# carry4985/ORB_SLAM2_MAP

Hardware: AMD Instinct MI355X
Metric: frames/sec ORB extract+match (640x480, 1000 feat) (higher is better)
Workload: dtype u8; 1 GPU; C2: synthetic 640x480 RGB-D stream, 1000 features, 8 levels, extract + BF-Hamming match of consecutive frames; resident_frame_pool=1024, sequences=1, parallelism=1 sequence per GPU, schedule_name=best, extraction_parts=1

## Files before the change

orb_slam2_map_amd/csrc/extractor.hip:

```cpp
#include "common.h"

#include <atomic>
#include <chrono>
#include <thread>
#include <tuple>
#include <type_traits>
#include <utility>
#include "trig_base.h"
#include "pyramid_view.h"
#include "extractor_plan.h"

#include <algorithm>
#include <cfloat>
#include <cmath>
#include <cstdlib>
#include <cstring>
#include <vector>

namespace orbgpu {

__host__ __device__ __forceinline__ uint32_t pack_key(int x, int y, int resp)
{
    return ((uint32_t)y << 20) | ((uint32_t)x << 8) | (uint32_t)resp;
}
// ... 1395 lines not shown
        best_done = last_pass;
        labelled = labelled || !last_pass;
        {
            int *t = S.ccnt;
            S.ccnt = S.ccnt_next;
            S.ccnt_next = t;
        }
        {
            short4 *tb = bndA; bndA = bndB; bndB = tb;
            int *tc = cntA; cntA = cntB; cntB = tc;
            uint16_t *tr = creA; creA = creB; creB = tr;
            uint32_t *tm = midA; midA = midB; midB = tm;
        }
        __syncthreads();
    }

    QT_MARK(3)
    const int n = n_cur;
    unsigned long long *best = reinterpret_cast<unsigned long long *>(S.ccnt);
    if (!best_done) {
        for (int p = tid; p < n; p += nt)
            best[p] = 0ull;
        __syncthreads();
        for (int i0 = tid; i0 < nkeys; i0 += QT_ILP * nt) {
            uint32_t key[QT_ILP];
            int nd[QT_ILP];
#pragma unroll
            for (int u = 0; u < QT_ILP; u++) {
                const int i = min(i0 + u * nt, nkeys - 1);
                key[u] = key_at(i);
                nd[u] = node_of(i, key[u]);
            }
#pragma unroll
            for (int u = 0; u < QT_ILP; u++)
                if (i0 + u * nt < nkeys)
                    atomicMax(&best[nd[u]], best_of(key[u]));
        }
    }
    __syncthreads();
    uint32_t *osel = sel + (size_t)f * sel_cap_total + g.sel_off;
    const bool ok = done_cur != 2 && n <= g.sel_cap;
    for (int p = tid; p < n && ok; p += nt) {
        const unsigned long long b = best[p];
        const uint32_t yx = (uint32_t)((0xFFFFFFFFFFull - (b & 0xFFFFFFFFFFull)) & 0xFFFFFFull);
        osel[p] = (yx << 8) | (uint32_t)((b >> 40) - 1ull);
    }
    QT_MARK(4)
    if (tid == 0)
        nsel[(size_t)f * nlevels + level] = ok ? n : -1;
}

struct KpAux {
    int x, y, level;
    float angle;
    float ca, sb;
    int plane_off, pitch;
};

__device__ __forceinline__ float fast_atan2_deg(float y, float x)
{
    const float s = (float)(180 / 3.14159265358979323846);
    const float p1 = 0.9997878412794807f * s, p3 = -0.3258083974640975f * s;
    const float p5 = 0.1555786518463281f * s, p7 = -0.04432655554792128f * s;
    const float ax = fabsf(x), ay = fabsf(y);
    float a, c, c2;
    if (ax >= ay) {
        c = ay / (ax + (float)DBL_EPSILON);
        c2 = c * c;
        a = (((p7 * c2 + p5) * c2 + p3) * c2 + p1) * c;
    } else {
        c = ax / (ay + (float)DBL_EPSILON);
        c2 = c * c;
        a = 90.f - (((p7 * c2 + p5) * c2 + p3) * c2 + p1) * c;
    }
    if (x < 0)
        a = 180.f - a;
    if (y < 0)
        a = 360.f - a;
    return a;
}

constexpr int OR_ITERS = 4;
constexpr int OR_BATCH_MIN = 32;

__global__ __launch_bounds__(256) void k_orient(const uint8_t *__restrict__ pyr, size_t frame_pyr,
                                                const LevelGeom *__restrict__ geom, int nlevels,
                                                const uint32_t *__restrict__ sel, int sel_cap_total,
                                                const int *__restrict__ nsel, const uint32_t *__restrict__ orw,
                                                orbgpu_keypoint *__restrict__ kps, KpAux *__restrict__ aux,
                                                int cap, int *__restrict__ n_out, int iters, Src0 s0)
{
    __shared__ uint32_t W10[4 * 16 * 9], M01[4 * 16 * 9];
    __shared__ __align__(16) uint8_t stage[8][31 * 48];
    for (int i = threadIdx.x; i < 4 * 16 * 9; i += 256) {
        W10[i] = orw[i];
        M01[i] = orw[4 * 16 * 9 + i];
    }
    __syncthreads();

    const int hl = threadIdx.x & 31;
    int bx, f;
    xcd_frame_block(bx, f);
    f = serpentine(f);
    const int *ns = nsel + (size_t)f * nlevels;
    for (int it = 0; it < iters; it++) {
    const int slot = (bx * iters + it) * 8 + (threadIdx.x >> 5);
    int level = -1, j = 0, out_off = 0, total = 0, cnt_l = 0;
    bool bad = false;
    struct {
        int plane_off, pitch, sel_off, patch;
        float scale;
    } g = {0, 0, 0, 0, 1.f};
    for (int l = 0; l < nlevels; l++) {
        const int c = ns[l];
        if (c < 0)
            bad = true;
        const int so = geom[l].sel_off;
        if (slot >= so && slot < so + geom[l].sel_cap) {
            level = l;
            j = slot - so;
            out_off = total;
            cnt_l = c;
            g.plane_off = geom[l].plane_off;
            g.pitch = geom[l].pitch;
            g.sel_off = so;
            g.patch = geom[l].patch;
            g.scale = geom[l].scale;
        }
        total += max(c, 0);
    }
    if (slot == 0 && hl == 0)
        n_out[f] = bad ? -1 - total : (total > cap ? -1 - total : total);
    if (level < 0 || bad || total > cap || j >= cnt_l)
        continue;
    const uint32_t key = sel[(size_t)f * sel_cap_total + g.sel_off + j];
    const int x = key_x(key) + BORDER0, y = key_y(key) + BORDER0;
    const bool dir0 = s0.direct != 0 && level == 0;
    const int porg = dir0 ? 0 : EDGE, ppitch = dir0 ? (int)s0.pitch : g.pitch;
    const int xl = x + porg - HALF_PATCH;
    const int a = xl & 3;
    const int v = hl - HALF_PATCH;
    int m10 = 0, m01 = 0;
    {
        const uint8_t *base = (dir0 ? s0.p + (size_t)f * s0.frame_stride : pyr + (size_t)f * frame_pyr + g.plane_off) + (xl - a);
        struct __attribute__((packed, aligned(4))) Piece {
            uint32_t d[4];
        };
        const int lim = a == 2 ? 3 : (a == 3 ? 6 : -1);
        const uint8_t *rowbase = base + rowoff(y + porg - HALF_PATCH, ppitch);
        uint4 *pl = reinterpret_cast<uint4 *>(stage[threadIdx.x >> 5]);
        Piece pc[3];
#pragma unroll
        for (int k = 0; k < 2; k++) {
            const int q = hl + 32 * k, r = q >> 1, part = q & 1;
            if (q < 62)
                pc[k] = *reinterpret_cast<const Piece *>(rowbase + rowoff(r, ppitch) + part * 16);
        }
        const int r2 = HALF_PATCH - lim + hl;
        if (hl < 2 * lim + 1)
            pc[2] = *reinterpret_cast<const Piece *>(rowbase + rowoff(r2, ppitch) + 32);
#pragma unroll
        for (int k = 0; k < 2; k++) {
            const int q = hl + 32 * k;
            if (q < 62)
                pl[3 * (q >> 1) + (q & 1)] = make_uint4(pc[k].d[0], pc[k].d[1], pc[k].d[2], pc[k].d[3]);
        }
        if (hl < 2 * lim + 1)
            pl[3 * r2 + 2] = make_uint4(pc[2].d[0], pc[2].d[1], pc[2].d[2], pc[2].d[3]);
        __builtin_amdgcn_fence(__ATOMIC_RELEASE, "wavefront");
        __builtin_amdgcn_wave_barrier();
        __builtin_amdgcn_fence(__ATOMIC_ACQUIRE, "wavefront");
        if (hl < 31) {
            const int av = v < 0 ? -v : v;
            const uint32_t *row = reinterpret_cast<const uint32_t *>(stage[threadIdx.x >> 5]) + hl * 12;
            const uint32_t *w = &W10[(a * 16 + av) * 9], *m = &M01[(a * 16 + av) * 9];
            uint32_t sw = 0, sm = 0;
#pragma unroll
            for (int q = 0; q < 9; q++) {
                const uint32_t d = row[q];
                sw = __builtin_amdgcn_udot4(d, w[q], sw, false);
                sm = __builtin_amdgcn_udot4(d, m[q], sm, false);
            }
            m10 = (int)sw - 16 * (int)sm;
            m01 = v * (int)sm;
        }
        __builtin_amdgcn_fence(__ATOMIC_RELEASE, "wavefront");
        __builtin_amdgcn_wave_barrier();
    }
#pragma unroll
    for (int off = 16; off > 0; off >>= 1) {
        m10 += __shfl_xor(m10, off, 64);
        m01 += __shfl_xor(m01, off, 64);
    }
    if (hl == 0) {
        const float angle = fast_atan2_deg((float)m01, (float)m10);
        orbgpu_keypoint kp;
        kp.x = (float)x;
        kp.y = (float)y;
        if (level != 0) {
            kp.x *= g.scale;
            kp.y *= g.scale;
        }
        kp.size = (float)g.patch;
        kp.angle = angle;
        kp.response = (float)key_resp(key);
        kp.octave = level;
        kp.class_id = -1;
        kps[(size_t)f * cap + out_off + j] = kp;
        KpAux ax;
        ax.x = x + (dir0 ? BLUR0_OX - EDGE : 0);
        ax.y = y;
        ax.level = level;
        ax.plane_off = g.plane_off;
        ax.pitch = g.pitch;
        ax.angle = angle;
        aux[(size_t)f * cap + out_off + j] = ax;
    }
    }
}
__global__ __launch_bounds__(256) void k_trig(KpAux *__restrict__ aux, const int *__restrict__ n_out, int cap, TrigTable tt)
{
    const int f = blockIdx.y;
    const int i = blockIdx.x * 256 + threadIdx.x;
    if (i >= n_out[f])
        return;
    KpAux *a = aux + (size_t)f * cap + i;
    const float factorPI = (float)(3.14159265358979323846 / 180.f);
    const float angle = a->angle * factorPI;
    float c, s;
    orbgpu_trig_device(angle, tt, &c, &s);
    a->ca = c;
    a->sb = s;
}

__device__ __forceinline__ void blur_hsum(uint32_t d0, uint32_t d1, uint32_t d2, uint32_t h[4])
{
#define W4(a, b, c, d) ((uint32_t)(a) | ((uint32_t)(b) << 8) | ((uint32_t)(c) << 16) | ((uint32_t)(d) << 24))
    h[0] = __builtin_amdgcn_udot4(d1, W4(55, 49, 34, 18), __builtin_amdgcn_udot4(d0, W4(0, 18, 34, 49), 0u, false), false);
    h[1] = __builtin_amdgcn_udot4(d2, W4(18, 0, 0, 0), __builtin_amdgcn_udot4(d1, W4(49, 55, 49, 34), __builtin_amdgcn_udot4(d0, W4(0, 0, 18, 34), 0u, false), false), false);
    h[2] = __builtin_amdgcn_udot4(d2, W4(34, 18, 0, 0), __builtin_amdgcn_udot4(d1, W4(34, 49, 55, 49), __builtin_amdgcn_udot4(d0, W4(0, 0, 0, 18), 0u, false), false), false);
    h[3] = __builtin_amdgcn_udot4(d2, W4(49, 34, 18, 0), __builtin_amdgcn_udot4(d1, W4(18, 34, 49, 55), 0u, false), false);
#undef W4
}

__device__ __forceinline__ uint32_t blur_vsum(const uint32_t A[4], const uint32_t C[4], const uint32_t E[4],
                                              const uint32_t F[4])
{
    const us2 K01 = {18, 34}, K23 = {49, 55}, K45 = {49, 34}, K6 = {0, 18};
    uint32_t sv[4];
#pragma unroll
    for (int p = 0; p < 4; p++) {
        uint32_t acc = __builtin_amdgcn_udot2(__builtin_bit_cast(us2, A[p]), K01, 32768u, false);
        acc = __builtin_amdgcn_udot2(__builtin_bit_cast(us2, C[p]), K23, acc, false);
        acc = __builtin_amdgcn_udot2(__builtin_bit_cast(us2, E[p]), K45, acc, false);
        sv[p] = __builtin_amdgcn_udot2(__builtin_bit_cast(us2, F[p]), K6, acc, false);
    }
    const us2 cap = {255, 255};
    const us2 lo = __builtin_elementwise_min(__builtin_bit_cast(us2, __builtin_amdgcn_perm(sv[1], sv[0], 0x07060302u)), cap);
    const us2 hi = __builtin_elementwise_min(__builtin_bit_cast(us2, __builtin_amdgcn_perm(sv[3], sv[2], 0x07060302u)), cap);
    return __builtin_amdgcn_perm(__builtin_bit_cast(uint32_t, hi), __builtin_bit_cast(uint32_t, lo), 0x06040200u);
}

__global__ __launch_bounds__(256) void k_blur(const uint8_t *__restrict__ pyr, uint8_t *__restrict__ blur,
                                               size_t frame_pyr, const LevelGeom *__restrict__ geom, StripGeom bg, int strip0)
{
    int bx, f;
    xcd_frame_block(bx, f);
    f = serpentine(f);
    const int strip = strip0 + bx * 256 + threadIdx.x;
    if (strip >= bg.first[bg.nlevels])
        return;
    int level = 0;
#pragma unroll
    for (int l = 1; l < ORBGPU_MAX_LEVELS; l++)
        level += (l < bg.nlevels && strip >= bg.first[l]) ? 1 : 0;
    const LevelGeom g = geom[level];
    const int local = strip - bg.first[level];
    const int sy = local / bg.nsx[level], sx = local - sy * bg.nsx[level];
    const int col = (4 + 2 * sx) * 4;
    const int y0 = sy * BLUR_ROWS;
    const int rows = min(BLUR_ROWS, g.h - y0);
    const uint8_t *fsrc = pyr + (size_t)f * frame_pyr;
    uint8_t *fdst = blur + (size_t)f * frame_pyr;
    const uint32_t pitch = (uint32_t)g.pitch;
    const uint32_t src0 = (uint32_t)g.plane_off + (uint32_t)(y0 + EDGE - 3) * pitch + (uint32_t)(col - 4);
    uint32_t soff = src0 + 6u * pitch;
    uint32_t doff = (uint32_t)g.plane_off + (uint32_t)(y0 + EDGE) * pitch + (uint32_t)col;
    struct __attribute__((packed, aligned(4))) Q4 {
        uint32_t d[4];
    };
    uint32_t p0[8], p1[8], p2[8], p3[8], p4[8], p5[8], hn[8];
    Q4 nx;
#define B8_HSUM(R, Q)                                                                                        \
    {                                                                                                        \
        blur_hsum(Q.d[0], Q.d[1], Q.d[2], R);                                                                \
        blur_hsum(Q.d[1], Q.d[2], Q.d[3], R + 4);                                                            \
    }
#define B8_PAIR(P, PREV, H)                                                                                  \
    _Pragma("unroll") for (int p = 0; p < 8; p++) P[p] = __builtin_amdgcn_alignbit(H[p], PREV[p], 16);
#define B8_LOAD(P, PREV, row)                                                                                \
// ... 528 lines not shown
        if (!direct) {
            int rcb = materialize_level0(e, s0, batch, L);
            if (rcb != ORBGPU_OK)
                return rcb;
        }
        for (int l = 1; l < nl; l++) {
            const LevelGeom &gl = e->plan.geom[l];
            const ResizeLaunch rl = resize_launch(e->plan, l, batch, direct);
            if (rl.px == 8) {
                dim3 gr8((resize_n8(gl.w) * ((gl.h + rl.rows - 1) / rl.rows) + 255) / 256, batch);
                L.launch(rl.dir1 ? (rl.share ? k_resize_fast<true, true, 8, true> : k_resize_fast<true, true, 8, false>)
                                 : (rl.share ? k_resize_fast<true, false, 8, true> : k_resize_fast<true, false, 8, false>), gr8, dim3(256), 0, pyr,
                         e->plan.frame_pyr, dg, l, e->tab<ResizeStrip>(e->plan.t_r8item), e->tab<uint4>(e->plan.t_r8sel), e->tab<uint4>(e->plan.t_r8wt),
                         e->tab<YRow>(e->plan.t_yrow), rl.off, rl.rows, s0);
            } else if (rl.px == 4) {
                dim3 grf((resize_ndw(gl.w) * ((gl.h + rl.rows - 1) / rl.rows) + 255) / 256, batch);
                auto kern = rl.dir1 ? (rl.rows == PYR_ROWS ? k_resize_fast<true, true, 4> : k_resize_fast<false, true, 4>)
                                    : (rl.rows == PYR_ROWS ? k_resize_fast<true, false, 4> : k_resize_fast<false, false, 4>);
                L.launch(kern, grf, dim3(256), 0, pyr, e->plan.frame_pyr, dg, l, e->tab<ResizeStrip>(e->plan.t_rstrip),
                                   e->tab<uint4>(e->plan.t_rsel), e->tab<uint4>(e->plan.t_rwt), e->tab<YRow>(e->plan.t_yrow),
                                   rl.off, rl.rows, s0);
            } else {
                dim3 gr((gl.pitch / 4 + 255) / 256, gl.h + 2 * EDGE, batch);
                L.launch(k_resize_level, gr, dim3(256), 0, pyr, e->plan.frame_pyr, dg, l,
                                   e->tab<XTab>(e->plan.t_xtab), e->tab<YTab>(e->plan.t_ytab));
            }
        }
    }
    END(ST_PYRAMID, st);
    BEGIN(ST_BLUR, st);
    if (side_blur) {
        ORBGPU_HIP_TRY(hipEventRecord(e->ev_fork, st));
        ORBGPU_HIP_TRY(hipStreamWaitEvent(e->side, e->ev_fork, 0));
        if (prof && !early_blur0)
            ORBGPU_HIP_TRY(hipEventRecord(evs[ST_COUNT + 1], e->side));
        launch_blur(e, s0, batch, Ls, early_blur0 ? 2 : 0);
        if (prof)
            ORBGPU_HIP_TRY(hipEventRecord(evs[ST_COUNT + 2], e->side));
        ORBGPU_HIP_TRY(hipEventRecord(e->ev_join, e->side));
    } else
        launch_blur(e, s0, batch, L);
    END(ST_BLUR, st);
    BEGIN(ST_FAST, st);
    if (e->counters_dirty) {
        int rcm = L.memset32(e->d_cellcnt.p, e->d_cellcnt.bytes & ~(size_t)3);
        if (rcm == ORBGPU_OK)
            rcm = L.memset32(e->d_qtaux.p, e->d_qtaux.bytes & ~(size_t)3);
        if (rcm != ORBGPU_OK)
            return rcm;
    }
    e->counters_dirty = true;
    {
        const int t_ini = std::max(e->prm.ini_th_fast, 1), t_min = std::max(e->prm.min_th_fast, 1);
        const DetectGeom &dgeo = direct ? e->plan.det_geom_direct : e->plan.det_geom;
        const int nwaves = (dgeo.first[nl] + FD_OWN - 1) / FD_OWN;
        L.launch(e->fast_early_out ? k_fast_detect<true> : k_fast_detect<false>, dim3((nwaves + 3) / 4, batch), dim3(256), 0, pyr, e->plan.frame_pyr, dg,
                           dgeo, e->tab<ColumnInfo>(e->plan.t_ctab), e->tab<CellDesc>(e->plan.t_cells), e->plan.ncells,
                           e->d_slots.as<uint32_t>(), e->plan.frame_slots, e->d_cellcnt.as<int>(), std::min(t_ini, t_min),
                           t_ini, e->fast_queue_cap, s0);
    }
    END(ST_FAST, st);
    BEGIN(ST_QUADTREE, st);
    {
        const QuadtreeLaunch ql = quadtree_launch(e->plan, batch, e->force_batch_quadtree);
        const bool pre = ql.lds_keys && e->plan.qt_prefilter;
        if (pre)
            L.launch(k_qt_prefilter, dim3(std::min((e->plan.max_slots_level + QT_PRE_KEYS - 1) / QT_PRE_KEYS, QT_PRE_GRID), nl, batch), dim3(256), 0, dg, e->plan.ncells, e->d_slots.as<uint32_t>(), e->plan.frame_slots, e->d_cellcnt.as<int>(),
                               e->d_dkey.as<uint32_t>(), e->d_qtaux.as<int>(), std::max(e->prm.ini_th_fast, 1));
        L.launch(ql.lds_keys ? k_quadtree<true> : k_quadtree<false>, dim3(batch, nl), dim3(ql.threads), ql.lds_bytes, dg,
                           e->tab<CellDesc>(e->plan.t_cells), e->plan.ncells, e->d_slots.as<uint32_t>(), e->plan.frame_slots,
                           e->d_cellcnt.as<int>(), e->d_dkey.as<uint32_t>(), e->d_dnode.as<uint16_t>(),
                           e->d_sel.as<uint32_t>(), e->plan.sel_cap_total, e->d_nsel.as<int>(), e->d_ncand.as<int>(), nl,
                           e->plan.ncap, std::max(e->prm.ini_th_fast, 1), ql.kcap, qt_dbg(),
                           pre ? e->d_qtaux.as<int>() : (int *)nullptr);
    }
    if (!rec)
        ORBGPU_HIP_TRY(hipGetLastError());
    e->counters_dirty = false;
    END(ST_QUADTREE, st);
    BEGIN(ST_ORIENT, st);
    const int or_iters = batch >= OR_BATCH_MIN ? OR_ITERS : 1;
    L.launch(k_orient, dim3((e->plan.sel_cap_total + 8 * or_iters - 1) / (8 * or_iters), batch), dim3(256), 0, pyr, e->plan.frame_pyr, dg, nl,
                       e->d_sel.as<uint32_t>(), e->plan.sel_cap_total, e->d_nsel.as<int>(),
                       e->tab<uint32_t>(e->plan.t_orient), d_kps,
                       e->d_aux.as<KpAux>(), cap, d_n_out, or_iters, s0);
    L.launch(k_trig, dim3((std::min(cap, e->plan.max_kp) + 255) / 256, batch), dim3(256), 0,
                       e->d_aux.as<KpAux>(), d_n_out, cap, e->trig);
    END(ST_ORIENT, st);
    BEGIN(ST_DESCRIBE, st);
    if (side_blur)
        ORBGPU_HIP_TRY(hipStreamWaitEvent(st, e->ev_join, 0));
    L.launch(k_describe, dim3((std::min(cap, e->plan.max_kp) + 7) / 8, batch), dim3(256), 0, blur,
                       e->plan.frame_pyr, dg, e->d_aux.as<KpAux>(), d_n_out, cap, e->tab<int8_t>(e->plan.t_pattern), d_desc);
    END(ST_DESCRIBE, st);
#undef BEGIN
#undef END
    if (!rec)
        ORBGPU_HIP_TRY(hipGetLastError());
    else if (L.err != hipSuccess) {
        set_error("recording the extraction graph: %s", hipGetErrorString(L.err));
        return ORBGPU_EHIP;
    }
    if (prof)
        e->prof_calls++;
    (void)w;
    (void)h;
    return ORBGPU_OK;
}

}

namespace orbgpu {

int extractor_pyramid_view(const orbgpu_extractor *e, PyramidView *v)
{
    ORBGPU_REQUIRE(e && v, "null argument");
    memset(v, 0, sizeof(*v));
    v->device_id = e->prm.device_id;
    v->nlevels = e->nlevels;
    v->scale_factor = e->prm.scale_factor;
    v->last_batch = (int)e->plan.geom.size() == e->nlevels ? e->last.batch : 0;
    for (int l = 0; l < e->nlevels; l++) {
        v->scale[l] = e->consts.scale[l];
        v->inv_scale[l] = e->consts.inv_scale[l];
        if (v->last_batch > 0) {
            const LevelGeom &g = e->plan.geom[l];
            v->w[l] = g.w;
            v->h[l] = g.h;
            v->pitch[l] = g.pitch;
            v->plane_off[l] = g.plane_off;
        }
    }
    v->pyr = e->d_pyr.as<uint8_t>();
    v->frame_pyr = e->plan.frame_pyr;
    v->border = EDGE;
    v->direct = v->last_batch > 0 && e->last.src.direct ? 1 : 0;
    v->l0 = v->direct ? e->last.src.p : nullptr;
    v->l0_frame_stride = v->direct ? e->last.src.frame_stride : 0;
    v->l0_pitch = v->direct ? e->last.src.pitch : 0;
    v->scratch = &e->d_stereo;
    return ORBGPU_OK;
}

}

extern "C" {

static void free_handle(orbgpu_extractor *e)
{
    for (DevBuf *b : e->buffers())
        b->release();
    for (auto &x : e->ev)
        if (x)
            (void)hipEventDestroy(x);
    if (e->graph_exec)
        (void)hipGraphExecDestroy(e->graph_exec);
    if (e->graph)
        (void)hipGraphDestroy(e->graph);
    if (e->h_pin)
        (void)hipHostFree(e->h_pin);
    if (e->stream)
        (void)hipStreamDestroy(e->stream);
    if (e->side)
        (void)hipStreamDestroy(e->side);
    if (e->ev_fork)
        (void)hipEventDestroy(e->ev_fork);
    if (e->ev_fork0)
// ... 642 lines not shown
```

orb_slam2_map_amd/csrc/extractor_plan.h:

```cpp
#pragma once
#include <algorithm>
#include <cmath>
#include <cstdarg>
#include <cstdint>
#include <cstdio>
#include <cstdlib>
#include <cstring>
#include <string>
#include <utility>
#include <vector>

#include "orbgpu.h"
#include "resize_tables.h"

#ifdef __HIPCC__
#define ORBGPU_PLAN_HD __host__ __device__ __forceinline__
#else
#define ORBGPU_PLAN_HD inline
#endif

namespace orbgpu {

constexpr int EDGE = 19;
static_assert(EDGE == RS_EDGE, "resize_tables.h builds its tables for this border");
// ... 149 lines not shown
        desired *= factor;
    }
    c->quota[nl - 1] = std::max(nfeatures - sum, 0);

    int *um = c->umax.v;
    const int vmax = (int)floor(HALF_PATCH * sqrtf(2.f) / 2 + 1);
    const int vmin = (int)ceil(HALF_PATCH * sqrtf(2.f) / 2);
    const double hp2 = HALF_PATCH * HALF_PATCH;
    for (int v = 0; v <= vmax; ++v)
        um[v] = cv_round_host(sqrt(hp2 - v * v));
    for (int v = HALF_PATCH, v0 = 0; v >= vmin; --v) {
        while (um[v0] == um[v0 + 1])
            ++v0;
        um[v] = v0;
        ++v0;
    }
    static const int expect[16] = {15, 15, 15, 15, 14, 14, 14, 13, 13, 12, 11, 10, 9, 8, 6, 3};
    for (int v = 0; v <= HALF_PATCH; v++)
        ORBGPU_PLAN_REQUIRE(um[v] == expect[v], "umax[%d] = %d, k_orient is written for %d", v, um[v], expect[v]);
    return ORBGPU_OK;
}

struct LevelSize {
    int w, h;
    float width, height;
};
inline LevelSize level_size(const ExtractorConsts &c, int w, int h, int l)
{
    LevelSize s;
    s.w = cv_round_host((float)w * c.inv_scale[l]);
    s.h = cv_round_host((float)h * c.inv_scale[l]);
    s.width = (float)(s.w - 2 * BORDER0);
    s.height = (float)(s.h - 2 * BORDER0);
    return s;
}
inline int level_n_ini(const LevelSize &s) { return (int)roundf(s.width / s.height); }
inline int level_max_keypoints(int n_ini, int quota) { return std::max(4 * n_ini, quota + 3); }

inline RingGeom ring_geom(const std::vector<LevelGeom> &geom, int ring)
{
    RingGeom rg = {};
    rg.nlevels = (int)geom.size();
    for (int l = 1; l < rg.nlevels; l++)
        rg.first[l + 1] = rg.first[l] + 2 * ring * (geom[l].w + 2 * ring) + 2 * ring * geom[l].h;
    return rg;
}

static const int8_t k_pattern_host[1024] = {
#include "orbgpu_pattern.inc"
};

struct PlanHooks {
    int qt_keys = -1;
    bool qt_no_prefilter = false;
};

struct PlanTable {
    size_t off = 0, bytes = 0;
};
constexpr size_t PLAN_ALIGN = 256;

struct ExtractorPlan {
    int w = 0, h = 0;
    std::vector<LevelGeom> geom;
    int ncells = 0;
    StripGeom blur_geom = {};
    DetectGeom det_geom = {}, det_geom_direct = {};
    RingGeom ring_full = {};
    size_t frame_pyr = 0, frame_slots = 0;
    int sel_cap_total = 0, ncap = 0, max_kp = 0;
    size_t qt_lds = 0;
    int qt_kcap = 0;
    int max_slots_level = 0;
    bool qt_prefilter = false;
    bool border_fast = false;
    bool direct0_ok = false;
    int rs_off_direct = 0;
    int r8_off[ORBGPU_MAX_LEVELS] = {};
    int r8_off_direct = -1;
    bool r8_share[ORBGPU_MAX_LEVELS] = {}, r8_share_direct = false;
    bool interior_resize = false;
    std::vector<uint8_t> blob;
    PlanTable t_geom, t_cells, t_ctab, t_bcol, t_xtab, t_ytab, t_yrow, t_rstrip, t_rsel, t_rwt, t_r8item, t_r8sel, t_r8wt,
        t_pattern, t_orient;
    template <typename T> const T *table(const PlanTable &t) const { return reinterpret_cast<const T *>(blob.data() + t.off); }
    template <typename T> size_t count(const PlanTable &t) const { return t.bytes / sizeof(T); }
};

template <typename T> inline PlanTable plan_add_table(std::vector<uint8_t> &blob, const T *data, size_t n)
{
    PlanTable t;
    t.off = (blob.size() + PLAN_ALIGN - 1) / PLAN_ALIGN * PLAN_ALIGN;
    t.bytes = n * sizeof(T);
    blob.resize(t.off + t.bytes, 0);
    if (t.bytes)
        memcpy(blob.data() + t.off, data, t.bytes);
    return t;
}

inline bool plan_detect(const std::vector<LevelGeom> &geom, bool direct0, DetectGeom &dgm, std::vector<ColumnInfo> &ctab)
{
    const int nl = (int)geom.size();
    memset(&dgm, 0, sizeof(dgm));
    dgm.nlevels = nl;
    int acc = 0;
    for (int l = 0; l < nl; l++) {
        const LevelGeom &g = geom[l];
        const bool dir = direct0 && l == 0;
        const int xfirst = dir ? 16 : 9 * 4 - EDGE;
        const int nsx = dir ? (g.w - 20 - xfirst) / 4 + 1 : (g.w - 1) / 4 - 9 + 1;
        const int nbands = (g.h - 2 * EDGE + g.hcell - 1) / g.hcell;
        dgm.first[l] = acc;
        dgm.nsx[l] = nsx;
        dgm.ncols[l] = g.ncols_eff;
        dgm.ctab_off[l] = (int)ctab.size();
        dgm.xfirst[l] = xfirst;
        acc += nsx * nbands;
        if (dir)
            acc = (acc + FD_OWN - 1) / FD_OWN * FD_OWN;
        for (int sx = 0; sx < nsx; sx++) {
            ColumnInfo c{0u, 0u};
            for (int p = 0; p < 4; p++) {
                const int x = xfirst + 4 * sx + p;
                int j = 0xFF;
                if (x >= EDGE && x < g.w - EDGE) {
                    j = (x - EDGE) / g.wcell;
                    const int xs = EDGE + j * g.wcell, xe = std::min(xs + g.wcell, g.w - EDGE);
                    if (j < g.ncols_eff) {
                        c.flags |= 1u << p;
                        if (x == xs)
                            c.flags |= 16u << p;
                        if (x == xe - 1)
                            c.flags |= 256u << p;
                    } else
                        j = 0xFF;
                }
                c.cellj |= (uint32_t)j << (8 * p);
            }
            ctab.push_back(c);
        }
    }
    for (int l = nl; l <= ORBGPU_MAX_LEVELS; l++)
        dgm.first[l] = acc;
    std::vector<std::pair<int, int>> strip_cells;
    for (int l = 0; l < nl; l++) {
        const LevelGeom &g = geom[l];
        const int nbands = (g.h - 2 * EDGE + g.hcell - 1) / g.hcell;
        strip_cells.resize((size_t)dgm.first[l], {-1, -1});
        for (int b = 0; b < nbands; b++)
            for (int sx = 0; sx < dgm.nsx[l]; sx++) {
                const ColumnInfo &c = ctab[dgm.ctab_off[l] + sx];
                int lo = -1, hi = -1;
                for (int p = 0; p < 4; p++)
                    if ((c.flags >> p) & 1u) {
                        const int id = g.cell_first + b * dgm.ncols[l] + (int)((c.cellj >> (8 * p)) & 255u);
                        lo = lo < 0 ? id : std::min(lo, id);
                        hi = std::max(hi, id);
                    }
                strip_cells.push_back({lo, hi});
            }
    }
    for (size_t w0 = 0; w0 < strip_cells.size(); w0 += FD_OWN) {
        int lo = -1, hi = -1;
        for (size_t q = w0; q < std::min(w0 + FD_OWN, strip_cells.size()); q++)
            if (strip_cells[q].first >= 0) {
                lo = lo < 0 ? strip_cells[q].first : std::min(lo, strip_cells[q].first);
                hi = std::max(hi, strip_cells[q].second);
            }
        if (hi - lo >= FD_CELLS)
            return false;
    }
    return true;
}

inline int plan_extractor(const ExtractorConsts &cst, int w, int h, const PlanHooks &hooks, ExtractorPlan *out,
                          std::string *why)
{
    ExtractorPlan &P = *out;
    P = ExtractorPlan();
    const int nl = cst.nlevels;
// ... 131 lines not shown
            const uint32_t m = (uint32_t)(((1ull << 32) + (uint64_t)d - 1u) / (uint64_t)d);
            for (uint32_t v = 0; v < 8192u; v++)
                ORBGPU_PLAN_REQUIRE((uint32_t)(((uint64_t)v * m) >> 32) == v / (uint32_t)d, "cell size %d at level %d has no exact reciprocal", d, l);
            (which ? g.inv_hcell : g.inv_wcell) = m;
        }
    }
    std::vector<ColumnInfo> ctab;
    ORBGPU_PLAN_REQUIRE(plan_detect(geom, false, P.det_geom, ctab),
                        "image too small for the FAST kernel's cell bookkeeping (more than %d cells in one wave)", FD_CELLS);
    if (direct_ok)
        direct_ok = plan_detect(geom, true, P.det_geom_direct, ctab);
    P.direct0_ok = direct_ok;
    P.rs_off_direct = rdirect.rs_off;
    for (int l = 0; l < ORBGPU_MAX_LEVELS; l++)
        P.r8_off[l] = l >= 1 && l < nl && rlev[l].fast8 ? rlev[l].r8_off : -1;
    P.r8_off_direct = direct_ok && rdirect.fast8 ? rdirect.r8_off : -1;
    for (int l = 0; l < ORBGPU_MAX_LEVELS; l++)
        P.r8_share[l] = l >= 1 && l < nl && rlev[l].share8;
    P.r8_share_direct = rdirect.share8;
    for (int l = 1; l < nl; l++)
        P.interior_resize = P.interior_resize || geom[l].rs_fast != 0;
    P.ring_full = ring_geom(geom, EDGE);
    std::vector<BorderCol> bcol;
    if (w % 4 == 0 && w >= 8) {
        const LevelGeom &g0 = geom[0];
        for (int c = 0; c < g0.pitch / 4; c++) {
            int sx[4], lo = 1 << 30, hi = 0;
            for (int k = 0; k < 4; k++) {
                sx[k] = reflect101(std::min(c * 4 + k, g0.w + 2 * EDGE - 1) - EDGE, g0.w);
                lo = std::min(lo, sx[k]);
                hi = std::max(hi, sx[k]);
            }
            const int d = std::min(lo / 4, g0.w / 4 - 2);
            ORBGPU_PLAN_REQUIRE(hi < d * 4 + 8 && lo >= d * 4, "level-0 border table: span of column %d", c);
            BorderCol bc{(uint32_t)d, 0u};
            for (int k = 0; k < 4; k++)
                bc.sel |= (uint32_t)(sx[k] - d * 4) << (8 * k);
            bcol.push_back(bc);
        }
    }
    P.border_fast = !bcol.empty();
    std::vector<uint32_t> orw(2 * 4 * 16 * 9, 0u);
    for (int i = 0; i < 4 * 16 * 9; i++) {
        const int a = i / (16 * 9), av = (i / 9) % 16, j = i % 9;
        for (int k = 0; k < 4; k++) {
            const int u = 4 * j + k - a - HALF_PATCH;
            if (std::abs(u) <= cst.umax.v[av]) {
                orw[i] |= (uint32_t)(u + 16) << (8 * k);
                orw[4 * 16 * 9 + i] |= 1u << (8 * k);
            }
        }
    }
    P.w = w;
    P.h = h;
    P.ncells = (int)cells.size();
    P.frame_pyr = plane_off;
    P.frame_slots = (size_t)slot_off;
    P.sel_cap_total = sel_off;
    P.ncap = ncap;
    P.qt_lds = qt_lds;
    P.qt_kcap = qt_kcap;
    P.max_slots_level = max_slots_level;
    P.qt_prefilter = !hooks.qt_no_prefilter;
    for (int l = 0; l < nl; l++) {
        P.qt_prefilter = P.qt_prefilter && geom[l].n_ini <= QT_INI_MAX;
        P.max_kp += geom[l].sel_cap - 1;
    }
    std::vector<uint8_t> &b = P.blob;
    P.t_geom = plan_add_table(b, geom.data(), geom.size());
    P.t_cells = plan_add_table(b, cells.data(), cells.size());
    P.t_ctab = plan_add_table(b, ctab.data(), ctab.size());
    P.t_bcol = plan_add_table(b, bcol.data(), bcol.size());
    P.t_xtab = plan_add_table(b, rt.xtab.data(), rt.xtab.size());
    P.t_ytab = plan_add_table(b, rt.ytab.data(), rt.ytab.size());
    P.t_yrow = plan_add_table(b, rt.yrow.data(), rt.yrow.size());
    P.t_rstrip = plan_add_table(b, rt.strip.data(), rt.strip.size());
    P.t_rsel = plan_add_table(b, rt.sel.data(), rt.sel.size());
    P.t_rwt = plan_add_table(b, rt.wt.data(), rt.wt.size());
    P.t_r8item = plan_add_table(b, rt.item8.data(), rt.item8.size());
    P.t_r8sel = plan_add_table(b, rt.sel8.data(), rt.sel8.size());
    P.t_r8wt = plan_add_table(b, rt.wt8.data(), rt.wt8.size());
    P.t_pattern = plan_add_table(b, k_pattern_host, sizeof(k_pattern_host));
    P.t_orient = plan_add_table(b, orw.data(), orw.size());
    return ORBGPU_OK;
}

struct QuadtreeLaunch {
    bool lds_keys;
    int kcap, threads;
    size_t lds_bytes;
};
inline QuadtreeLaunch quadtree_launch(const ExtractorPlan &p, int batch, bool force_batch_variant)
{
    if (batch >= QT_BATCH_MIN || force_batch_variant)
        return QuadtreeLaunch{false, 0, QT_THREADS_BATCH, p.qt_lds};
    return QuadtreeLaunch{true, p.qt_kcap, p.w * p.h >= QT_LARGE_PIXELS ? QT_THREADS : QT_THREADS_SMALL,
                          p.qt_lds + (size_t)p.qt_kcap * 6};
}

struct ResizeLaunch {
    int px;
    int rows;
    bool share;
    bool dir1;
    int off;
};
inline ResizeLaunch resize_launch(const ExtractorPlan &p, int l, int batch, bool direct)
{
    const LevelGeom &g = p.geom[l];
    if (!g.rs_fast)
        return ResizeLaunch{0, 0, false, false, 0};
    const bool dir1 = direct && l == 1;
    const int r8 = batch >= PYR_BATCH_MIN ? (dir1 ? p.r8_off_direct : p.r8_off[l]) : -1;
    if (r8 >= 0)
        return ResizeLaunch{8, PYR_ROWS, dir1 ? p.r8_share_direct : p.r8_share[l], dir1, r8};
    const int ndw_l = (g.pitch / 4) * (g.h + 2 * EDGE);
    const int rows = batch >= PYR_BATCH_MIN || ndw_l >= 32768 ? PYR_ROWS : ndw_l >= 16384 ? PYR_ROWS / 2 : PYR_ROWS / 4;
    return ResizeLaunch{4, rows, false, dir1, dir1 ? p.rs_off_direct : g.rs_off};
}

}
```

Measured before the change: 313,000 frames/s.

## Precompute per-level orientation metadata once per block and batch keypoint loads

k_orient now builds a shared per-level table (sel offset, count, output offset via wave prefix sum, plane geometry) once per block. Previously every wave iteration looped over all levels reading geom and nsel. A host-built slot-to-level byte table lets each lane fetch one keypoint's level and key up front, and these are broadcast with shuffles across iterations. The W10/M01 weights are interleaved into one 16-byte-aligned LDS array so they can be read as vector loads. The cross-lane reduction now uses DPP/swizzle, and results are written once per lane after the loop. The change adds LDS use and a __syncthreads, and changes how the early-exit and n_out paths are handled.

```diff
diff --git a/orb_slam2_map_amd/csrc/extractor.hip b/orb_slam2_map_amd/csrc/extractor.hip
--- a/orb_slam2_map_amd/csrc/extractor.hip
+++ b/orb_slam2_map_amd/csrc/extractor.hip
@@ -1501,58 +1501,110 @@
 
 constexpr int OR_ITERS = 4;
 constexpr int OR_BATCH_MIN = 32;
+struct OrientLevel {
+    int sel_off, cnt;
+    int out_off;
+    int plane_off, pitch, patch;
+    float scale;
+    int pad;
+};
+static_assert(sizeof(OrientLevel) == 32, "OrientLevel is read as two 16-byte words");
+
+__device__ __forceinline__ int or_sum32(int v)
+{
+    v += __builtin_amdgcn_update_dpp(0, v, 0xB1, 0xF, 0xF, false);
+    v += __builtin_amdgcn_update_dpp(0, v, 0x4E, 0xF, 0xF, false);
+    v += __builtin_amdgcn_update_dpp(0, v, 0x124, 0xF, 0xF, false);
+    v += __builtin_amdgcn_update_dpp(0, v, 0x128, 0xF, 0xF, false);
+    return v + __builtin_amdgcn_ds_swizzle(v, 0x401F);
+}
 
 __global__ __launch_bounds__(256) void k_orient(const uint8_t *__restrict__ pyr, size_t frame_pyr,
                                                 const LevelGeom *__restrict__ geom, int nlevels,
                                                 const uint32_t *__restrict__ sel, int sel_cap_total,
                                                 const int *__restrict__ nsel, const uint32_t *__restrict__ orw,
+                                                const uint8_t *__restrict__ slot_lev,
                                                 orbgpu_keypoint *__restrict__ kps, KpAux *__restrict__ aux,
                                                 int cap, int *__restrict__ n_out, int iters, Src0 s0)
 {
-    __shared__ uint32_t W10[4 * 16 * 9], M01[4 * 16 * 9];
+    constexpr int OR_WM = 20;
+    __shared__ __align__(16) uint32_t WM[4 * 16 * OR_WM];
     __shared__ __align__(16) uint8_t stage[8][31 * 48];
-    for (int i = threadIdx.x; i < 4 * 16 * 9; i += 256) {
-        W10[i] = orw[i];
-        M01[i] = orw[4 * 16 * 9 + i];
-    }
-    __syncthreads();
-
-    const int hl = threadIdx.x & 31;
+    __shared__ __align__(16) OrientLevel lev[ORBGPU_MAX_LEVELS];
+    __shared__ int s_total, s_bad;
     int bx, f;
     xcd_frame_block(bx, f);
     f = serpentine(f);
-    const int *ns = nsel + (size_t)f * nlevels;
+    {
+        const int row = threadIdx.x >> 2, part = threadIdx.x & 3;
+#pragma unroll
+        for (int k = 0; k < 3; k++) {
+            const int q = part + 4 * k;
+            if (q < 9) {
+                WM[row * OR_WM + 2 * q] = orw[row * 9 + q];
+                WM[row * OR_WM + 2 * q + 1] = orw[4 * 16 * 9 + row * 9 + q];
+            }
+        }
+    }
+    static_assert(ORBGPU_MAX_LEVELS <= 16, "the prefix sum below covers 16 lanes");
+    if (threadIdx.x < 64) {
+        const int l = threadIdx.x;
+        const bool has = l < nlevels;
+        const int c = has ? nsel[(size_t)f * nlevels + l] : 0;
+        const int pos = max(c, 0);
+        int incl = pos;
+#pragma unroll
+        for (int off = 1; off < 16; off <<= 1) {
+            const int t = __shfl_up(incl, off, 64);
+            if (l >= off)
+                incl += t;
+        }
+        const bool bad = __ballot(c < 0) != 0;
+        if (has) {
+            const LevelGeom &G = geom[l];
+            OrientLevel r;
+            r.sel_off = G.sel_off;
+            r.cnt = c;
+            r.out_off = incl - pos;
+            r.plane_off = G.plane_off;
+            r.pitch = G.pitch;
+            r.patch = G.patch;
+            r.scale = G.scale;
+            r.pad = 0;
+            lev[l] = r;
+            if (l == nlevels - 1) {
+                s_total = incl;
+                s_bad = bad ? 1 : 0;
+            }
+        }
+    }
+    __syncthreads();
+
+    const int hl = threadIdx.x & 31;
+    const int half = threadIdx.x >> 5;
+    const int total = s_total;
+    const bool bad = s_bad != 0;
+    if (bx == 0 && threadIdx.x == 0)
+        n_out[f] = bad ? -1 - total : (total > cap ? -1 - total : total);
+    if (bad || total > cap)
+        return;
+    int my_level = -1;
+    uint32_t my_key = 0;
+    const int my_slot = (bx * iters + hl) * 8 + half;
+    if (hl < iters && my_slot < sel_cap_total) {
+        const int l = slot_lev[my_slot];
+        my_key = sel[(size_t)f * sel_cap_total + my_slot];
+        my_level = my_slot - lev[l].sel_off < lev[l].cnt ? l : -1;
+    }
+    int my_m10 = 0, my_m01 = 0;
     for (int it = 0; it < iters; it++) {
-    const int slot = (bx * iters + it) * 8 + (threadIdx.x >> 5);
-    int level = -1, j = 0, out_off = 0, total = 0, cnt_l = 0;
-    bool bad = false;
+    const int level = __shfl(my_level, it, 32);
+    const uint32_t key = __shfl(my_key, it, 32);
+    if (level < 0)
+        continue;
     struct {
-        int plane_off, pitch, sel_off, patch;
-        float scale;
-    } g = {0, 0, 0, 0, 1.f};
-    for (int l = 0; l < nlevels; l++) {
-        const int c = ns[l];
-        if (c < 0)
-            bad = true;
-        const int so = geom[l].sel_off;
-        if (slot >= so && slot < so + geom[l].sel_cap) {
-            level = l;
-            j = slot - so;
-            out_off = total;
-            cnt_l = c;
-            g.plane_off = geom[l].plane_off;
-            g.pitch = geom[l].pitch;
-            g.sel_off = so;
-            g.patch = geom[l].patch;
-            g.scale = geom[l].scale;
-        }
-        total += max(c, 0);
-    }
-    if (slot == 0 && hl == 0)
-        n_out[f] = bad ? -1 - total : (total > cap ? -1 - total : total);
-    if (level < 0 || bad || total > cap || j >= cnt_l)
-        continue;
-    const uint32_t key = sel[(size_t)f * sel_cap_total + g.sel_off + j];
+        int plane_off, pitch;
+    } g = {lev[level].plane_off, lev[level].pitch};
     const int x = key_x(key) + BORDER0, y = key_y(key) + BORDER0;
     const bool dir0 = s0.direct != 0 && level == 0;
     const int porg = dir0 ? 0 : EDGE, ppitch = dir0 ? (int)s0.pitch : g.pitch;
@@ -1592,13 +1644,17 @@
         if (hl < 31) {
             const int av = v < 0 ? -v : v;
             const uint32_t *row = reinterpret_cast<const uint32_t *>(stage[threadIdx.x >> 5]) + hl * 12;
-            const uint32_t *w = &W10[(a * 16 + av) * 9], *m = &M01[(a * 16 + av) * 9];
+            const uint4 *wm4 = reinterpret_cast<const uint4 *>(&WM[(a * 16 + av) * OR_WM]);
+            const uint4 p0 = wm4[0], p1 = wm4[1], p2 = wm4[2], p3 = wm4[3];
+            const uint2 p4 = *reinterpret_cast<const uint2 *>(&wm4[4]);
+            const uint32_t wm[18] = {p0.x, p0.y, p0.z, p0.w, p1.x, p1.y, p1.z, p1.w, p2.x,
+                                     p2.y, p2.z, p2.w, p3.x, p3.y, p3.z, p3.w, p4.x, p4.y};
             uint32_t sw = 0, sm = 0;
 #pragma unroll
             for (int q = 0; q < 9; q++) {
                 const uint32_t d = row[q];
-                sw = __builtin_amdgcn_udot4(d, w[q], sw, false);
-                sm = __builtin_amdgcn_udot4(d, m[q], sm, false);
+                sw = __builtin_amdgcn_udot4(d, wm[2 * q], sw, false);
+                sm = __builtin_amdgcn_udot4(d, wm[2 * q + 1], sm, false);
             }
             m10 = (int)sw - 16 * (int)sm;
             m01 = v * (int)sm;
@@ -1606,35 +1662,41 @@
         __builtin_amdgcn_fence(__ATOMIC_RELEASE, "wavefront");
         __builtin_amdgcn_wave_barrier();
     }
-#pragma unroll
-    for (int off = 16; off > 0; off >>= 1) {
-        m10 += __shfl_xor(m10, off, 64);
-        m01 += __shfl_xor(m01, off, 64);
-    }
-    if (hl == 0) {
-        const float angle = fast_atan2_deg((float)m01, (float)m10);
+    m10 = or_sum32(m10);
+    m01 = or_sum32(m01);
+    if (hl == it) {
+        my_m10 = m10;
+        my_m01 = m01;
+    }
+    }
+    if (my_level >= 0) {
+        const int level = my_level;
+        const OrientLevel my = lev[level];
+        const int my_j = my_slot - my.sel_off;
+        const int x = key_x(my_key) + BORDER0, y = key_y(my_key) + BORDER0;
+        const bool dir0 = s0.direct != 0 && level == 0;
+        const float angle = fast_atan2_deg((float)my_m01, (float)my_m10);
         orbgpu_keypoint kp;
         kp.x = (float)x;
         kp.y = (float)y;
         if (level != 0) {
-            kp.x *= g.scale;
-            kp.y *= g.scale;
-        }
-        kp.size = (float)g.patch;
+            kp.x *= my.scale;
+            kp.y *= my.scale;
+        }
+        kp.size = (float)my.patch;
         kp.angle = angle;
-        kp.response = (float)key_resp(key);
+        kp.response = (float)key_resp(my_key);
         kp.octave = level;
         kp.class_id = -1;
-        kps[(size_t)f * cap + out_off + j] = kp;
+        kps[(size_t)f * cap + my.out_off + my_j] = kp;
         KpAux ax;
         ax.x = x + (dir0 ? BLUR0_OX - EDGE : 0);
         ax.y = y;
         ax.level = level;
-        ax.plane_off = g.plane_off;
-        ax.pitch = g.pitch;
+        ax.plane_off = my.plane_off;
+        ax.pitch = my.pitch;
         ax.angle = angle;
-        aux[(size_t)f * cap + out_off + j] = ax;
-    }
+        aux[(size_t)f * cap + my.out_off + my_j] = ax;
     }
 }
 __global__ __launch_bounds__(256) void k_trig(KpAux *__restrict__ aux, const int *__restrict__ n_out, int cap, TrigTable tt)
@@ -2329,7 +2391,7 @@
     const int or_iters = batch >= OR_BATCH_MIN ? OR_ITERS : 1;
     L.launch(k_orient, dim3((e->plan.sel_cap_total + 8 * or_iters - 1) / (8 * or_iters), batch), dim3(256), 0, pyr, e->plan.frame_pyr, dg, nl,
                        e->d_sel.as<uint32_t>(), e->plan.sel_cap_total, e->d_nsel.as<int>(),
-                       e->tab<uint32_t>(e->plan.t_orient), d_kps,
+                       e->tab<uint32_t>(e->plan.t_orient), e->tab<uint8_t>(e->plan.t_slot_level), d_kps,
                        e->d_aux.as<KpAux>(), cap, d_n_out, or_iters, s0);
     L.launch(k_trig, dim3((std::min(cap, e->plan.max_kp) + 255) / 256, batch), dim3(256), 0,
                        e->d_aux.as<KpAux>(), d_n_out, cap, e->trig);
diff --git a/orb_slam2_map_amd/csrc/extractor_plan.h b/orb_slam2_map_amd/csrc/extractor_plan.h
--- a/orb_slam2_map_amd/csrc/extractor_plan.h
+++ b/orb_slam2_map_amd/csrc/extractor_plan.h
@@ -255,7 +255,7 @@
     bool interior_resize = false;
     std::vector<uint8_t> blob;
     PlanTable t_geom, t_cells, t_ctab, t_bcol, t_xtab, t_ytab, t_yrow, t_rstrip, t_rsel, t_rwt, t_r8item, t_r8sel, t_r8wt,
-        t_pattern, t_orient;
+        t_pattern, t_orient, t_slot_level;
     template <typename T> const T *table(const PlanTable &t) const { return reinterpret_cast<const T *>(blob.data() + t.off); }
     template <typename T> size_t count(const PlanTable &t) const { return t.bytes / sizeof(T); }
 };
@@ -269,6 +269,16 @@
     if (t.bytes)
         memcpy(blob.data() + t.off, data, t.bytes);
     return t;
+}
+
+inline int slot_level(const std::vector<LevelGeom> &geom, int slot)
+{
+    if (slot < 0 || geom.empty() || slot >= geom.back().sel_off + geom.back().sel_cap)
+        return -1;
+    int level = 0;
+    for (size_t l = 1; l < geom.size(); l++)
+        level += slot >= geom[l].sel_off ? 1 : 0;
+    return level;
 }
 
 inline bool plan_detect(const std::vector<LevelGeom> &geom, bool direct0, DetectGeom &dgm, std::vector<ColumnInfo> &ctab)
@@ -566,6 +576,10 @@
     P.t_r8wt = plan_add_table(b, rt.wt8.data(), rt.wt8.size());
     P.t_pattern = plan_add_table(b, k_pattern_host, sizeof(k_pattern_host));
     P.t_orient = plan_add_table(b, orw.data(), orw.size());
+    std::vector<uint8_t> slot_lev((size_t)sel_off);
+    for (int s = 0; s < sel_off; s++)
+        slot_lev[(size_t)s] = (uint8_t)slot_level(geom, s);
+    P.t_slot_level = plan_add_table(b, slot_lev.data(), slot_lev.size());
     return ORBGPU_OK;
 }
 
```

Result: faster. 317,200 frames/s, median of 6 (+1.4%).
